# AlejandroSilvestri/os1

Measured on AMD Instinct MI355X. Metric: frames/sec extract+match, 1920x1080 @ 2000 ORB feats, higher is better.
Workload: dtype u8

## Files before the change

### os1_amd/csrc/orbfe_fast.hip

```cpp
#include <hip/hip_runtime.h>

#include <algorithm>
#include <cstdlib>
#include <type_traits>
#include <vector>

#include "orbfe_internal.h"

namespace orbfe {

namespace {
__device__ __forceinline__ int m24(int a, int b) { return __mul24(a, b); }
typedef unsigned short u16x2 __attribute__((ext_vector_type(2)));
__device__ __forceinline__ u16x2 as_u16x2(unsigned v) { return __builtin_bit_cast(u16x2, v); }
__device__ __forceinline__ unsigned as_u32(u16x2 v) { return __builtin_bit_cast(unsigned, v); }
}

__device__ __forceinline__ unsigned pk_min3_h(unsigned a, unsigned b, unsigned c) {
  unsigned r;
  asm("v_pk_minimum3_f16 %0, %1, %2, %3" : "=v"(r) : "v"(a), "v"(b), "v"(c));
  return r;
}
__device__ __forceinline__ unsigned pk_max3_h(unsigned a, unsigned b, unsigned c) {
  unsigned r;
  asm("v_pk_maximum3_f16 %0, %1, %2, %3" : "=v"(r) : "v"(a), "v"(b), "v"(c));
  return r;
}

__device__ __forceinline__ void wave_lds_fence() { asm volatile("s_waitcnt lgkmcnt(0)" ::: "memory"); }

struct FastArgs {
  const FastCell* cells;
  const uint8_t* const* frame0;
  const uint8_t* frameInline[2];
  long long stride0;
  uint8_t* slab;
  long long slabBytes;
  uint32_t* cellCount;
  uint32_t* slots;
  long long slotsPerFrame;
  const uint8_t* zeros;
  int ncells, pad, iniTh, minTh, frameBase;
};
static FastArgs fast_args(const PyramidParams& P) {
  FastArgs A{};
  A.cells = P.cells; A.frame0 = P.frame0; A.frameInline[0] = P.frameInline[0]; A.frameInline[1] = P.frameInline[1];
  A.stride0 = P.stride0; A.slab = P.slab; A.slabBytes = P.slabBytes; A.cellCount = P.cellCount; A.slots = P.slots;
  A.slotsPerFrame = P.slotsPerFrame; A.zeros = P.zeros; A.ncells = P.ncells; A.iniTh = P.iniTh; A.minTh = P.minTh;
  A.frameBase = P.frameBase;
  return A;
}

__device__ uint32_t* g_fastStampBuf;
template <int ABL = 0, bool LEAN = false>
__global__ __launch_bounds__(64) __attribute__((amdgpu_num_sgpr(96))) void k_fast_tasks(FastArgs P, int cb, int nc) {
  extern __shared__ __align__(16) uint8_t lds[];
  unsigned long long stamp[6] = {0, 0, 0, 0, 0, 0};
  if constexpr (ABL == 4) stamp[0] = __builtin_amdgcn_s_memtime();
  asm volatile("" ::"s"(P.cells), "s"(P.frame0), "s"(P.frameInline[0]), "s"(P.frameInline[1]), "s"(P.stride0), "s"(P.slab), "s"(P.slabBytes),
               "s"(P.cellCount), "s"(P.slots), "s"(P.slotsPerFrame), "s"(P.zeros), "s"(P.ncells), "s"(P.iniTh), "s"(P.minTh), "s"(P.frameBase),
               "s"(cb), "s"(nc));
  const int chunk = (nc + 7) >> 3;
  const int cloc = (blockIdx.x & 7) * chunk + (blockIdx.x >> 3);
  if (cloc >= nc) return;
  const int cix = cb + cloc;
  const int f = P.frameBase + blockIdx.y;
  const int lane = threadIdx.x;
  typedef uint32_t u32x8 __attribute__((ext_vector_type(8)));
  typedef uint32_t u32x2 __attribute__((ext_vector_type(2)));
  const u32x8 tw = *reinterpret_cast<const u32x8 __attribute__((address_space(4)))*>(reinterpret_cast<uintptr_t>(P.cells + cix));
  u32x2 fpw;
  if (P.frame0) {
    fpw = *reinterpret_cast<const u32x2 __attribute__((address_space(4)))*>(reinterpret_cast<uintptr_t>(P.frame0 + f));
  } else {
    const unsigned long long v = reinterpret_cast<unsigned long long>((f & 1) ? P.frameInline[1] : P.frameInline[0]);
    fpw.x = (uint32_t)v;
    fpw.y = (uint32_t)(v >> 32);
  }
  const int ex0 = (int)(tw[0] & 0xffffu), ey0 = (int)(tw[0] >> 16);
  const int ew = (int)(tw[1] & 0xffu), eh = (int)((tw[1] >> 16) & 0xffu), level = (int)(tw[1] >> 24);
  const uint32_t cell = tw[2], slotOff = tw[3], roiOff = tw[4], pitchL = tw[5];
  const int wCell = (int)(tw[6] & 0xffu), hCell = (int)((tw[6] >> 8) & 0xffu);
  uint32_t* cnt;
  if constexpr (LEAN) cnt = reinterpret_cast<uint32_t*>(reinterpret_cast<uint8_t*>(P.cellCount) + 4u * ((uint32_t)f * (uint32_t)P.ncells + cell));
  else cnt = P.cellCount + (long long)f * P.ncells + cell;
  if (ew == 0) {
    if (lane == 0) cnt[0] = 0;
    return;
  }
  long long stride;
  const uint8_t* roi;
  if constexpr (LEAN) {
    const bool l0 = level == 0;
    const uint32_t st32 = l0 ? (uint32_t)P.stride0 : pitchL;
    const uint32_t off = l0 ? (uint32_t)(ey0 - 3) * st32 + (uint32_t)(ex0 - 3) : (uint32_t)f * (uint32_t)P.slabBytes + roiOff;
    const uint8_t* base = l0 ? reinterpret_cast<const uint8_t*>(((unsigned long long)fpw.y << 32) | fpw.x) : P.slab;
    stride = (long long)st32;
    roi = base + off;
  } else if (level == 0) {
    stride = P.stride0;
    roi = reinterpret_cast<const uint8_t*>(((unsigned long long)fpw.y << 32) | fpw.x) + (long long)(ey0 - 3) * stride + (ex0 - 3);
  } else {
    stride = (long long)pitchL;
    roi = P.slab + (long long)f * P.slabBytes + roiOff;
  }
  const uint32_t geo = tw[7];
  const int TP = LEAN ? (int)(geo & 7u) << 4 : ((wCell + 6 + 3 + 15) & ~15);
  const int SP = wCell + 2;
  uint8_t* tile = lds;
  const int scOff = LEAN ? (int)((geo >> 8) & 0x3ffu) << 4 : (TP * (hCell + 6) + 15) & ~15;
  uint8_t* sc = tile + scOff;
  uint16_t* queue = reinterpret_cast<uint16_t*>(lds + (LEAN ? (int)((geo >> 18) & 0x7ffu) << 4 : ((scOff + SP * (hCell + 2) + 15) & ~15)));

  const int rw = ew + 6, rh = eh + 6;
  const int istr = (int)stride;
  const int a = (int)(reinterpret_cast<uintptr_t>(roi) & 3);
  if constexpr (ABL == 4) { asm volatile("" ::"s"(a), "s"(istr), "s"(TP) : "memory"); stamp[1] = __builtin_amdgcn_s_memtime(); }
  if constexpr (LEAN) {
    const int ppr = (int)(geo & 7u), rpi = (int)((geo >> 3) & 31u);
    const float rn = __builtin_amdgcn_rcpf((float)ppr);
    const int lrow = (int)(((float)lane + 0.5f) * rn), lcol = lane - m24(lrow, ppr);
    const bool on = lrow < rpi && 16 * lcol < a + rw;
    const unsigned voff = (unsigned)(m24(lrow, istr) + 16 * lcol);
    const uint8_t* gp = roi - a;
    const uint32_t gstep = (uint32_t)rpi * (uint32_t)istr;
    const int lstep = rpi * TP;
    uint8_t* lp = tile;
#pragma nounroll
    for (int left = rh; left > 0; left -= rpi, gp += gstep, lp += lstep) {
      unsigned vo = voff;
      asm volatile("" : "+s"(gp), "+v"(vo));
      if (on && lrow < left)
        __builtin_amdgcn_global_load_lds((const __attribute__((address_space(1))) void*)(gp + vo),
                                         (__attribute__((address_space(3))) void*)lp, 16, 0, 0);
    }
  } else if ((stride & 3) == 0) {
    const int ppr = TP >> 4;
    const float rn = __builtin_amdgcn_rcpf((float)ppr);
    const int rpi = 64 / ppr;
    const int lrow = (int)(((float)lane + 0.5f) * rn), lcol = lane - m24(lrow, ppr);
    const bool on = lrow < rpi && 16 * lcol < a + rw;
    const unsigned voff = (unsigned)(m24(lrow, istr) + 16 * lcol);
    const uint8_t* gp = roi - a;
    const long long gstep = (long long)rpi * stride;
    const int lstep = m24(rpi, TP);
    uint8_t* lp = tile;
    for (int left = rh; left > 0; left -= rpi, gp += gstep, lp += lstep) {
      unsigned vo = voff;
      asm volatile("" : "+s"(gp), "+v"(vo));
      if (on && lrow < left)
        __builtin_amdgcn_global_load_lds((const __attribute__((address_space(1))) void*)(gp + vo),
                                         (__attribute__((address_space(3))) void*)lp, 16, 0, 0);
    }
  } else {
    const float rcpRw = 1.0f / (float)rw;
    const int total = rw * rh;
    for (int i0 = lane; i0 < total; i0 += 64 * 8) {
      uint8_t v[8];
#pragma unroll
      for (int u = 0; u < 8; u++) {
        const int i = i0 + u * 64;
        v[u] = 0;
        if (i < total) {
          const int y = (int)(((float)i + 0.5f) * rcpRw), x = i - m24(y, rw);
          v[u] = roi[m24(y, istr) + x];
        }
      }
#pragma unroll
      for (int u = 0; u < 8; u++) {
        const int i = i0 + u * 64;
        if (i < total) {
          const int y = (int)(((float)i + 0.5f) * rcpRw), x = i - m24(y, rw);
          tile[m24(y, TP) + a + x] = v[u];
        }
      }
    }
  }
  tile += a;
  if constexpr (LEAN) {
    const int pieces = (SP * (eh + 2) + 15) >> 4;
#pragma nounroll
    for (int p0 = 0; p0 < pieces; p0 += 64)
      if (lane < pieces - p0)
        __builtin_amdgcn_global_load_lds((const __attribute__((address_space(1))) void*)P.zeros,
                                         (__attribute__((address_space(3))) void*)(sc + 16 * p0), 16, 0, 0);
  } else {
    const int pieces = (SP * (eh + 2) + 15) >> 4;
    for (int p0 = 0; p0 < pieces; p0 += 64)
      if (lane < pieces - p0)
        __builtin_amdgcn_global_load_lds((const __attribute__((address_space(1))) void*)P.zeros,
                                         (__attribute__((address_space(3))) void*)(sc + 16 * p0), 16, 0, 0);
  }
  asm volatile("s_waitcnt vmcnt(0)" ::: "memory");
  wave_lds_fence();
  if constexpr (ABL == 4) stamp[2] = __builtin_amdgcn_s_memtime();
  if constexpr (ABL == 1) {
    unsigned acc = 0;
    for (int i = lane; i < (TP * rh) >> 2; i += 64) acc ^= reinterpret_cast<const uint32_t*>(tile - a)[i];
    if (acc == 0x9e3779b9u && lane == 63) cnt[0] = 0;
    if (lane == 0) cnt[0] = 0;
    return;
  }

  const unsigned long long below = (1ull << lane) - 1ull;
  uint32_t* slot;
  if constexpr (LEAN) slot = reinterpret_cast<uint32_t*>(reinterpret_cast<uint8_t*>(P.slots) + 4u * ((uint32_t)f * (uint32_t)P.slotsPerFrame + slotOff));
  else slot = P.slots + (long long)f * P.slotsPerFrame + slotOff;
  int base = 0;
  for (int pass = 0; pass < 2; pass++) {
    const int tlo = pass ? P.minTh : P.iniTh;
    int nq = 0;
    constexpr int NPX = 16, GS = 4, NS = 4;
    const int G = (ew + NPX - 1) >> GS, nItems = G * eh;
    const int stepY = (int)((0x10152040u >> ((G - 1) << 3)) & 0xffu), stepG = 64 - stepY * G;
    auto stage1 = [&](auto aTag) {
      constexpr int A = decltype(aTag)::value;
      const u16x2 T2 = as_u16x2((unsigned)tlo * 0x01000100u);
      auto test4 = [&](uint32_t L4, uint32_t C4, uint32_t R4, uint32_t U4, uint32_t D4, unsigned& fe, unsigned& fo) {
        unsigned flag[2];
#pragma unroll
        for (int h = 0; h < 2; h++) {
          const u16x2 v2 = h ? as_u16x2(C4) << 8 : as_u16x2(C4);
          const u16x2 r0 = h ? as_u16x2(D4) << 8 : as_u16x2(D4), r4 = h ? as_u16x2(R4) << 8 : as_u16x2(R4);
          const u16x2 r8 = h ? as_u16x2(U4) << 8 : as_u16x2(U4), r12 = h ? as_u16x2(L4) << 8 : as_u16x2(L4);
          const u16x2 mx = __builtin_elementwise_min(__builtin_elementwise_max(r0, r8), __builtin_elementwise_max(r4, r12));
          const u16x2 mn = __builtin_elementwise_max(__builtin_elementwise_min(r0, r8), __builtin_elementwise_min(r4, r12));
          const u16x2 dd = __builtin_elementwise_max(__builtin_elementwise_sub_sat(mx, v2), __builtin_elementwise_sub_sat(v2, mn));
          const unsigned e = as_u32(__builtin_elementwise_sub_sat(dd, T2));
          asm("v_pk_min_u16 %0, %1, %2" : "=v"(flag[h]) : "v"(e), "v"(0x00010001u));
        }
        fo = flag[0];
        fe = flag[1];
      };
      int y = (int)(((float)lane + 0.5f) * __builtin_amdgcn_rcpf((float)G)), g = lane - m24(y, G);
      int ro = m24(y, TP) + (g << GS);
      const int roStep = m24(stepY, TP) + (stepG << GS), roCarry = TP - (G << GS);
      const uint8_t* tb = tile - a;
      for (int i0 = 0; i0 < nItems; i0 += 64) {
        unsigned m = 0;
        if (i0 + lane < nItems) {
          constexpr int c0 = (A + 3) >> 2, cs = (A + 3) & 3, q0 = (A + 6) >> 2, qs = (A + 6) & 3;
          const uint32_t* cw = reinterpret_cast<const uint32_t*>(tb + 3 * TP + ro);
          uint32_t w[NS + 3];
#pragma unroll
          for (int k = 0; k < NS + 3; k++) w[k] = cw[k];
          const uint32_t* uw = reinterpret_cast<const uint32_t*>(tb + ro) + c0;
          const uint32_t* dw = reinterpret_cast<const uint32_t*>(tb + 6 * TP + ro) + c0;
          uint32_t u[NS + 1], d[NS + 1];
#pragma unroll
          for (int k = 0; k < NS + 1; k++) { u[k] = uw[k]; d[k] = dw[k]; }
          unsigned E = 0, O = 0;
#pragma unroll
          for (int j = 0; j < NS; j++) {
            const uint32_t Lj = __builtin_amdgcn_alignbyte(w[j + 1], w[j], A);
            const uint32_t Cj = __builtin_amdgcn_alignbyte(w[c0 + j + 1], w[c0 + j], cs);
            const uint32_t Rj = __builtin_amdgcn_alignbyte(w[q0 + j + 1], w[q0 + j], qs);
            const uint32_t Uj = __builtin_amdgcn_alignbyte(u[j + 1], u[j], cs);
            const uint32_t Dj = __builtin_amdgcn_alignbyte(d[j + 1], d[j], cs);
            unsigned fe, fo;
            test4(Lj, Cj, Rj, Uj, Dj, fe, fo);
            E |= fe << (4 * j);
            O |= fo << (4 * j);
          }
          const unsigned T = E | (O << 1);
          const int rem = ew - (g << GS);
          m = (T | (T >> 14)) & ((1u << min(rem, NPX)) - 1u);
        }
        const int c = __popc(m);
        int incl = c;
        incl += __builtin_amdgcn_update_dpp(0, incl, 0x111, 0xf, 0xf, true);
        incl += __builtin_amdgcn_update_dpp(0, incl, 0x112, 0xf, 0xf, true);
        incl += __builtin_amdgcn_update_dpp(0, incl, 0x114, 0xf, 0xf, true);
        incl += __builtin_amdgcn_update_dpp(0, incl, 0x118, 0xf, 0xf, true);
        incl += __builtin_amdgcn_update_dpp(0, incl, 0x142, 0xa, 0xf, false);
        incl += __builtin_amdgcn_update_dpp(0, incl, 0x143, 0xc, 0xf, false);
        const int pos = nq + incl - c;
        const unsigned e = (unsigned)((y << 8) | (g << GS));
        {
          unsigned rev = __builtin_bitreverse32(m), ent = e;
          unsigned addr = (unsigned)(uintptr_t)(queue + pos);
          unsigned long long saved;
          asm volatile(
              "s_mov_b64 %3, exec\n\t"
              ".rept %4\n\t"
              "v_add_co_u32 %0, vcc, %0, %0\n\t"
              "s_and_b64 exec, %3, vcc\n\t"
              "ds_write_b16 %1, %2\n\t"
              "v_add_u32 %1, 2, %1\n\t"
              "s_mov_b64 exec, %3\n\t"
              "v_add_u32 %2, 1, %2\n\t"
              ".endr"
              : "+v"(rev), "+v"(addr), "+v"(ent), "=&s"(saved)
              : "n"(NPX)
              : "vcc", "scc", "memory");
        }
        nq += __builtin_amdgcn_readlane(incl, 63);
        if (i0 + 64 >= nItems) break;
        y += stepY;
        g += stepG;
        ro += roStep;
        if (g >= G) { g -= G; y++; ro += roCarry; }
      }
    };
    switch (a) {
      case 0: stage1(std::integral_constant<int, 0>{}); break;
      case 1: stage1(std::integral_constant<int, 1>{}); break;
      case 2: stage1(std::integral_constant<int, 2>{}); break;
      default: stage1(std::integral_constant<int, 3>{}); break;
    }
    wave_lds_fence();
    if constexpr (ABL == 4) { if (pass == 0) stamp[3] = __builtin_amdgcn_s_memtime(); }
    if constexpr (ABL == 2) {
      unsigned acc = 0;
      for (int i = lane; i < nq; i += 64) acc ^= queue[i];
      if (lane == 0) cnt[0] = (acc == 0xffffffffu) ? 1u : 0u;
      return;
    }
    int nq2 = 0;
    for (int i0 = 0; i0 < nq; i0 += 64) {
      const int i = i0 + lane;
      bool ok = false;
      unsigned e = 0;
      if (i < nq) {
        e = queue[i];
        const int y = e >> 8, x = e & 0xff;
        const uint8_t* c = tile + m24(y + 3, TP) + (x + 3);
        const unsigned vv = c[0];
        constexpr unsigned B = 2048u;
        unsigned xr[16];
        const unsigned VV = (B + vv) | ((B - vv) << 16);
#define RING(k, off) asm("v_pk_mad_i16 %0, %1, %2, %3 op_sel_hi:[0,1,1]" : "=v"(xr[k]) : "v"((unsigned)c[off]), "v"(0x0001ffffu), "v"(VV));
        RING(0, 3 * TP);       RING(1, 3 * TP + 1);   RING(2, 2 * TP + 2);    RING(3, TP + 3);
        RING(4, 3);            RING(5, -TP + 3);      RING(6, -2 * TP + 2);   RING(7, -3 * TP + 1);
        RING(8, -3 * TP);      RING(9, -3 * TP - 1);  RING(10, -2 * TP - 2);  RING(11, -TP - 3);
        RING(12, -3);          RING(13, TP - 3);      RING(14, 2 * TP - 2);   RING(15, 3 * TP - 1);
#undef RING
        unsigned t[16], arc[16];
#pragma unroll
        for (int k = 0; k < 16; k++) t[k] = pk_min3_h(xr[k], xr[(k + 1) & 15], xr[(k + 2) & 15]);
#pragma unroll
        for (int k = 0; k < 16; k++) arc[k] = pk_min3_h(t[k], t[(k + 3) & 15], t[(k + 6) & 15]);
        const unsigned m0 = pk_max3_h(arc[0], arc[1], arc[2]), m1 = pk_max3_h(arc[3], arc[4], arc[5]), m2 = pk_max3_h(arc[6], arc[7], arc[8]);
        const unsigned m3 = pk_max3_h(arc[9], arc[10], arc[11]), m4 = pk_max3_h(arc[12], arc[13], arc[14]);
        const unsigned best = pk_max3_h(pk_max3_h(m0, m1, m2), pk_max3_h(m3, m4, arc[15]), arc[15]);
        const int S = (int)max(best & 0xffffu, best >> 16) - (int)B;
        ok = S > tlo;
        if (ok) sc[m24(y + 1, SP) + (x + 1)] = (uint8_t)(S - 1);
      }
      const unsigned long long mk = __ballot(ok);
      if (ok) queue[nq2 + __popcll(mk & below)] = (uint16_t)e;
      nq2 += __popcll(mk);
    }
    wave_lds_fence();
    if constexpr (ABL == 4) { if (pass == 0) stamp[4] = __builtin_amdgcn_s_memtime(); }
    if constexpr (ABL == 3) {
      unsigned acc = 0;
      for (int i = lane; i < nq2; i += 64) acc ^= queue[i] ^ sc[i];
      if (lane == 0) cnt[0] = (acc == 0xffffffffu) ? 1u : 0u;
      return;
    }
    for (int i0 = 0; i0 < nq2; i0 += 64) {
      const int i = i0 + lane;
      int keep = 0, y = 0, x = 0;
      if (i < nq2) {
        const unsigned e = queue[i];
        y = e >> 8;
        x = e & 0xff;
        const uint8_t* q = sc + m24(y + 1, SP) + (x + 1);
        const int sv = q[0];
        const int nmax = max(max(max((int)q[-1], (int)q[-SP - 1]), (int)q[SP - 1]), max(max(max((int)q[1], (int)q[-SP + 1]), (int)q[SP + 1]), max((int)q[-SP], (int)q[SP])));
        if (sv > nmax) keep = sv;
      }
      const uint32_t rec = (uint32_t)(ex0 + x) | ((uint32_t)(ey0 + y) << 12) | ((uint32_t)keep << 24);
      const unsigned long long mk = __ballot(keep > 0);
      if (keep > 0) slot[base + __popcll(mk & below)] = rec;
      base += __popcll(mk);
    }
    if (pass == 1 || P.minTh == P.iniTh) break;
    if constexpr (ABL == 5) break;
    if (base != 0) break;
    wave_lds_fence();
  }
  if (lane == 0) cnt[0] = (uint32_t)base;
  if constexpr (ABL == 4) {
    stamp[5] = __builtin_amdgcn_s_memtime();
    if (lane == 0 && g_fastStampBuf) {
      uint32_t* rec = g_fastStampBuf + 8ull * ((unsigned long long)blockIdx.y * (P.ncells + 64) + cix);
      for (int k = 0; k < 5; k++) rec[k] = (uint32_t)(stamp[k + 1] - stamp[k]);
      rec[5] = 1u;
    }
  }
}

#ifdef ORBFE_EXPERIMENTS
static uint32_t* s_stampBuf = nullptr;
static size_t s_stampWaves = 0;
int fast_stamps(unsigned long long out[8], int reset) {
  for (int k = 0; k < 8; k++) out[k] = 0;
  if (!s_stampBuf || !s_stampWaves) return 0;
  std::vector<uint32_t> h(8 * s_stampWaves);
  if (hipMemcpy(h.data(), s_stampBuf, h.size() * 4, hipMemcpyDeviceToHost) != hipSuccess) return 1;
  for (size_t w = 0; w < s_stampWaves; w++)
    if (h[8 * w + 5]) {
      for (int k = 0; k < 5; k++) out[k] += h[8 * w + k];
      out[5]++;
    }
  if (reset && hipMemset(s_stampBuf, 0, h.size() * 4) != hipSuccess) return 1;
  return 0;
}
static void stamp_buffer_for(size_t waves) {
  if (waves > s_stampWaves) {
    if (s_stampBuf) (void)hipFree(s_stampBuf);
    s_stampBuf = nullptr;
    if (hipMalloc((void**)&s_stampBuf, waves * 32) != hipSuccess) { s_stampWaves = 0; return; }
    s_stampWaves = waves;
    (void)hipMemcpyToSymbol(HIP_SYMBOL(g_fastStampBuf), &s_stampBuf, sizeof s_stampBuf);
  }
  (void)hipMemset(s_stampBuf, 0, s_stampWaves * 32);
}
#else
int fast_stamps(unsigned long long out[8], int) {
  for (int k = 0; k < 8; k++) out[k] = 0;
  return 1;
}
#endif

static size_t fast_lds_bytes_level(const LevelGeom& L) {
  const size_t TP = (size_t)((L.wCell + 6 + 3 + 15) & ~15);
  const size_t scOff = (TP * (L.hCell + 6) + 15) & ~(size_t)15;
  const size_t b = ((scOff + (size_t)(L.wCell + 2) * (L.hCell + 2) + 15) & ~(size_t)15) +
                   2 * (size_t)L.wCell * L.hCell + 64;
  return (b + 15) & ~(size_t)15;
}
uint32_t fast_cell_geo(int wCell, int hCell) {
  const uint32_t TP = (uint32_t)((wCell + 6 + 3 + 15) & ~15), ppr = TP >> 4;
  if (ppr == 0 || ppr > 7) return 0u;
  const uint32_t rpi = 64u / ppr;
  const uint32_t scOff = (TP * (uint32_t)(hCell + 6) + 15u) & ~15u;
  const uint32_t qOff = (scOff + (uint32_t)(wCell + 2) * (uint32_t)(hCell + 2) + 15u) & ~15u;
  if (rpi > 31u || (scOff >> 4) > 0x3ffu || (qOff >> 4) > 0x7ffu) return 0u;
  return ppr | (rpi << 3) | ((scOff >> 4) << 8) | ((qOff >> 4) << 18);
}

void launch_fast(const PyramidParams& P, int nframes, hipStream_t st) {
  const FastArgs FA = fast_args(P);
  const int level0 = 0, level1 = P.nlevels;
  constexpr size_t kLdsFull = 5120;
  static const int leanEnv = [] { const char* e = getenv("ORBFE_FAST_LEAN"); return e ? atoi(e) : 1; }();
#ifdef ORBFE_EXPERIMENTS
  static const int ablate = [] { const char* e = ORBFE_EXP_ENV("ORBFE_FAST_ABLATE"); return e ? atoi(e) : 0; }();
#endif
  int l = level0;
  while (l < level1) {
    int e = l + 1;
    size_t need = fast_lds_bytes_level(P.lv[l]);
    if (nframes > 2) {
      const bool small = need <= kLdsFull;
      while (e < level1 && (fast_lds_bytes_level(P.lv[e]) <= kLdsFull) == small) { need = std::max(need, fast_lds_bytes_level(P.lv[e])); e++; }
    } else {
      while (e < level1) { need = std::max(need, fast_lds_bytes_level(P.lv[e])); e++; }
    }
    const int cb = P.lv[l].cellBase, nc = (e < P.nlevels ? P.lv[e].cellBase : P.ncells) - cb;
    l = e;
    if (nc <= 0) continue;
    const dim3 grid(8 * ((nc + 7) / 8), nframes);
    const unsigned long long frames = (unsigned long long)P.frameBase + (unsigned long long)nframes;
    const bool lean = leanEnv && P.fastLean && P.zeros && (P.stride0 & 3) == 0 && P.stride0 > 0 && P.stride0 < (1ll << 31) &&
                      frames * (unsigned long long)P.slabBytes < (1ull << 32) && frames * (unsigned long long)P.slotsPerFrame * 4ull < (1ull << 32) &&
                      frames * (unsigned long long)P.ncells * 4ull < (1ull << 32) &&
                      (unsigned long long)P.lv[0].h * (unsigned long long)P.stride0 < (1ull << 32);
#ifdef ORBFE_EXPERIMENTS
    if (ablate) {
      if (ablate == 4 && cb == 0) stamp_buffer_for((size_t)(P.ncells + 64) * nframes);
#define ORBFE_FAST_ABL(A)                                                                                              \
  do {                                                                                                                 \
    if (lean) hipLaunchKernelGGL((k_fast_tasks<A, true>), grid, dim3(64), need, st, FA, cb, nc);                       \
    else hipLaunchKernelGGL((k_fast_tasks<A, false>), grid, dim3(64), need, st, FA, cb, nc);                           \
  } while (0)
      switch (ablate) {
        case 1: ORBFE_FAST_ABL(1); break;
        case 2: ORBFE_FAST_ABL(2); break;
        case 3: ORBFE_FAST_ABL(3); break;
        case 4: ORBFE_FAST_ABL(4); break;
        default: ORBFE_FAST_ABL(5); break;
      }
#undef ORBFE_FAST_ABL
      continue;
    }
#endif
    if (lean) hipLaunchKernelGGL((k_fast_tasks<0, true>), grid, dim3(64), need, st, FA, cb, nc);
    else hipLaunchKernelGGL((k_fast_tasks<0, false>), grid, dim3(64), need, st, FA, cb, nc);
  }
}

}
```

Before: 89530.

## Pair FAST cells per two-wave block and pool tail scoring across waves

```diff
diff --git a/os1_amd/csrc/fast_pool_plan.h b/os1_amd/csrc/fast_pool_plan.h
--- /dev/null
+++ b/os1_amd/csrc/fast_pool_plan.h
@@ -0,0 +1,43 @@
+#pragma once
+
+#if defined(__HIPCC__) || defined(__CUDACC__)
+#define ORBFE_FAST_POOL_HD __host__ __device__
+#else
+#define ORBFE_FAST_POOL_HD
+#endif
+
+namespace orbfe {
+
+constexpr int kFastTrip = 64;
+enum FastPoolMode { kFastPoolNone = 0, kFastPoolPooled = 1, kFastPoolSeparate = 2 };
+
+struct FastPoolPlan {
+  int mode;
+  int la, lb;
+  int runner;
+  int sync;
+};
+
+ORBFE_FAST_POOL_HD inline FastPoolPlan fast_pool_plan(int nqA, int nqB) {
+  FastPoolPlan p;
+  p.la = nqA > kFastTrip ? nqA - kFastTrip : 0;
+  p.lb = nqB > kFastTrip ? nqB - kFastTrip : 0;
+  const int sum = p.la + p.lb;
+  p.mode = sum == 0 ? kFastPoolNone : sum <= kFastTrip ? kFastPoolPooled : kFastPoolSeparate;
+  p.sync = (p.mode == kFastPoolPooled && p.la > 0 && p.lb > 0) ? 1 : 0;
+  p.runner = (p.mode == kFastPoolPooled && p.la == 0) ? 1 : 0;
+  return p;
+}
+
+ORBFE_FAST_POOL_HD inline int fast_pool_own_end(const FastPoolPlan& p, int wave, int nq) {
+  if (p.mode == kFastPoolPooled && (p.sync || p.runner != wave)) return nq < kFastTrip ? nq : kFastTrip;
+  return nq;
+}
+
+ORBFE_FAST_POOL_HD inline bool fast_pool_lane(const FastPoolPlan& p, int lane, int& cell, int& entry) {
+  if (lane < p.la) { cell = 0; entry = kFastTrip + lane; return true; }
+  if (lane < p.la + p.lb) { cell = 1; entry = kFastTrip + lane - p.la; return true; }
+  return false;
+}
+
+}
diff --git a/os1_amd/csrc/orbfe_fast.hip b/os1_amd/csrc/orbfe_fast.hip
--- a/os1_amd/csrc/orbfe_fast.hip
+++ b/os1_amd/csrc/orbfe_fast.hip
@@ -5,6 +5,7 @@
 #include <type_traits>
 #include <vector>
 
+#include "fast_pool_plan.h"
 #include "orbfe_internal.h"
 
 namespace orbfe {
@@ -28,6 +29,7 @@
 }
 
 __device__ __forceinline__ void wave_lds_fence() { asm volatile("s_waitcnt lgkmcnt(0)" ::: "memory"); }
+__device__ __forceinline__ void block_sync() { asm volatile("s_waitcnt lgkmcnt(0)\n\ts_barrier" ::: "memory"); }
 
 struct FastArgs {
   const FastCell* cells;
@@ -53,19 +55,23 @@
 
 __device__ uint32_t* g_fastStampBuf;
 template <int ABL = 0, bool LEAN = false>
-__global__ __launch_bounds__(64) __attribute__((amdgpu_num_sgpr(96))) void k_fast_tasks(FastArgs P, int cb, int nc) {
+__global__ __launch_bounds__(128) __attribute__((amdgpu_num_sgpr(96))) void k_fast_tasks(FastArgs P, int cb, int nc, int need) {
   extern __shared__ __align__(16) uint8_t lds[];
   unsigned long long stamp[6] = {0, 0, 0, 0, 0, 0};
   if constexpr (ABL == 4) stamp[0] = __builtin_amdgcn_s_memtime();
   asm volatile("" ::"s"(P.cells), "s"(P.frame0), "s"(P.frameInline[0]), "s"(P.frameInline[1]), "s"(P.stride0), "s"(P.slab), "s"(P.slabBytes),
                "s"(P.cellCount), "s"(P.slots), "s"(P.slotsPerFrame), "s"(P.zeros), "s"(P.ncells), "s"(P.iniTh), "s"(P.minTh), "s"(P.frameBase),
-               "s"(cb), "s"(nc));
-  const int chunk = (nc + 7) >> 3;
-  const int cloc = (blockIdx.x & 7) * chunk + (blockIdx.x >> 3);
-  if (cloc >= nc) return;
-  const int cix = cb + cloc;
+               "s"(cb), "s"(nc), "s"(need));
+  const int np = (nc + 1) >> 1;
+  const int chunk = (np + 7) >> 3;
+  const int ploc = (blockIdx.x & 7) * chunk + (blockIdx.x >> 3);
+  if (ploc >= np) return;
+  const int wv = __builtin_amdgcn_readfirstlane((int)(threadIdx.x >> 6));
+  const int cloc = 2 * ploc + wv;
+  const bool have = cloc < nc;
+  const int cix = cb + (have ? cloc : nc - 1);
   const int f = P.frameBase + blockIdx.y;
-  const int lane = threadIdx.x;
+  const int lane = threadIdx.x & 63;
   typedef uint32_t u32x8 __attribute__((ext_vector_type(8)));
   typedef uint32_t u32x2 __attribute__((ext_vector_type(2)));
   const u32x8 tw = *reinterpret_cast<const u32x8 __attribute__((address_space(4)))*>(reinterpret_cast<uintptr_t>(P.cells + cix));
@@ -84,10 +90,7 @@
   uint32_t* cnt;
   if constexpr (LEAN) cnt = reinterpret_cast<uint32_t*>(reinterpret_cast<uint8_t*>(P.cellCount) + 4u * ((uint32_t)f * (uint32_t)P.ncells + cell));
   else cnt = P.cellCount + (long long)f * P.ncells + cell;
-  if (ew == 0) {
-    if (lane == 0) cnt[0] = 0;
-    return;
-  }
+  const bool active = have && ew != 0;
   long long stride;
   const uint8_t* roi;
   if constexpr (LEAN) {
@@ -107,16 +110,19 @@
   const uint32_t geo = tw[7];
   const int TP = LEAN ? (int)(geo & 7u) << 4 : ((wCell + 6 + 3 + 15) & ~15);
   const int SP = wCell + 2;
-  uint8_t* tile = lds;
+  uint8_t* const half = lds + wv * need;
+  uint32_t* const mbox = reinterpret_cast<uint32_t*>(lds + 2 * need);
+  uint8_t* tile = half;
   const int scOff = LEAN ? (int)((geo >> 8) & 0x3ffu) << 4 : (TP * (hCell + 6) + 15) & ~15;
   uint8_t* sc = tile + scOff;
-  uint16_t* queue = reinterpret_cast<uint16_t*>(lds + (LEAN ? (int)((geo >> 18) & 0x7ffu) << 4 : ((scOff + SP * (hCell + 2) + 15) & ~15)));
+  uint16_t* queue = reinterpret_cast<uint16_t*>(half + (LEAN ? (int)((geo >> 18) & 0x7ffu) << 4 : ((scOff + SP * (hCell + 2) + 15) & ~15)));
 
   const int rw = ew + 6, rh = eh + 6;
   const int istr = (int)stride;
   const int a = (int)(reinterpret_cast<uintptr_t>(roi) & 3);
   if constexpr (ABL == 4) { asm volatile("" ::"s"(a), "s"(istr), "s"(TP) : "memory"); stamp[1] = __builtin_amdgcn_s_memtime(); }
-  if constexpr (LEAN) {
+  if (!active) {
+  } else if constexpr (LEAN) {
     const int ppr = (int)(geo & 7u), rpi = (int)((geo >> 3) & 31u);
     const float rn = __builtin_amdgcn_rcpf((float)ppr);
     const int lrow = (int)(((float)lane + 0.5f) * rn), lcol = lane - m24(lrow, ppr);
@@ -177,7 +183,8 @@
     }
   }
   tile += a;
-  if constexpr (LEAN) {
+  if (!active) {
+  } else if constexpr (LEAN) {
     const int pieces = (SP * (eh + 2) + 15) >> 4;
 #pragma nounroll
     for (int p0 = 0; p0 < pieces; p0 += 64)
@@ -196,10 +203,18 @@
   if constexpr (ABL == 4) stamp[2] = __builtin_amdgcn_s_memtime();
   if constexpr (ABL == 1) {
     unsigned acc = 0;
-    for (int i = lane; i < (TP * rh) >> 2; i += 64) acc ^= reinterpret_cast<const uint32_t*>(tile - a)[i];
-    if (acc == 0x9e3779b9u && lane == 63) cnt[0] = 0;
-    if (lane == 0) cnt[0] = 0;
+    if (active)
+      for (int i = lane; i < (TP * rh) >> 2; i += 64) acc ^= reinterpret_cast<const uint32_t*>(tile - a)[i];
+    if (have && acc == 0x9e3779b9u && lane == 63) cnt[0] = 0;
+    if (have && lane == 0) cnt[0] = 0;
     return;
+  }
+  if (wv == 1 && lane == 0) {
+    mbox[8 + 3] = (uint32_t)(tile - lds);
+    mbox[8 + 4] = (uint32_t)TP;
+    mbox[8 + 5] = (uint32_t)(sc - lds);
+    mbox[8 + 6] = (uint32_t)SP;
+    mbox[8 + 7] = (uint32_t)(reinterpret_cast<uint8_t*>(queue) - lds);
   }
 
   const unsigned long long below = (1ull << lane) - 1ull;
@@ -207,12 +222,13 @@
   if constexpr (LEAN) slot = reinterpret_cast<uint32_t*>(reinterpret_cast<uint8_t*>(P.slots) + 4u * ((uint32_t)f * (uint32_t)P.slotsPerFrame + slotOff));
   else slot = P.slots + (long long)f * P.slotsPerFrame + slotOff;
   int base = 0;
+  bool mine = active;
   for (int pass = 0; pass < 2; pass++) {
     const int tlo = pass ? P.minTh : P.iniTh;
     int nq = 0;
     constexpr int NPX = 16, GS = 4, NS = 4;
     const int G = (ew + NPX - 1) >> GS, nItems = G * eh;
-    const int stepY = (int)((0x10152040u >> ((G - 1) << 3)) & 0xffu), stepG = 64 - stepY * G;
+    const int stepY = (int)((0x10152040u >> (((G - 1) & 3) << 3)) & 0xffu), stepG = 64 - stepY * G;
     auto stage1 = [&](auto aTag) {
       constexpr int A = decltype(aTag)::value;
       const u16x2 T2 = as_u16x2((unsigned)tlo * 0x01000100u);
@@ -302,7 +318,7 @@
         if (g >= G) { g -= G; y++; ro += roCarry; }
       }
     };
-    switch (a) {
+    if (mine) switch (a) {
       case 0: stage1(std::integral_constant<int, 0>{}); break;
       case 1: stage1(std::integral_constant<int, 1>{}); break;
       case 2: stage1(std::integral_constant<int, 2>{}); break;
@@ -313,50 +329,85 @@
     if constexpr (ABL == 2) {
       unsigned acc = 0;
       for (int i = lane; i < nq; i += 64) acc ^= queue[i];
-      if (lane == 0) cnt[0] = (acc == 0xffffffffu) ? 1u : 0u;
+      if (have && lane == 0) cnt[0] = (acc == 0xffffffffu) ? 1u : 0u;
       return;
     }
+    if (lane == 0) mbox[8 * wv] = (uint32_t)nq;
+    block_sync();
+    const int nqOther = __builtin_amdgcn_readfirstlane((int)mbox[8 * (wv ^ 1)]);
+    const FastPoolPlan plan = fast_pool_plan(wv ? nqOther : nq, wv ? nq : nqOther);
+    auto score = [&](unsigned e, const uint8_t* tl, int tp, uint8_t* scb, int sp) -> bool {
+      const int y = e >> 8, x = e & 0xff;
+      const uint8_t* c = tl + m24(y + 3, tp) + (x + 3);
+      const unsigned vv = c[0];
+      constexpr unsigned B = 2048u;
+      unsigned xr[16];
+      const unsigned VV = (B + vv) | ((B - vv) << 16);
+#define RING(k, off) asm("v_pk_mad_i16 %0, %1, %2, %3 op_sel_hi:[0,1,1]" : "=v"(xr[k]) : "v"((unsigned)c[off]), "v"(0x0001ffffu), "v"(VV));
+      RING(0, 3 * tp);       RING(1, 3 * tp + 1);   RING(2, 2 * tp + 2);    RING(3, tp + 3);
+      RING(4, 3);            RING(5, -tp + 3);      RING(6, -2 * tp + 2);   RING(7, -3 * tp + 1);
+      RING(8, -3 * tp);      RING(9, -3 * tp - 1);  RING(10, -2 * tp - 2);  RING(11, -tp - 3);
+      RING(12, -3);          RING(13, tp - 3);      RING(14, 2 * tp - 2);   RING(15, 3 * tp - 1);
+#undef RING
+      unsigned t[16], arc[16];
+#pragma unroll
+      for (int k = 0; k < 16; k++) t[k] = pk_min3_h(xr[k], xr[(k + 1) & 15], xr[(k + 2) & 15]);
+#pragma unroll
+      for (int k = 0; k < 16; k++) arc[k] = pk_min3_h(t[k], t[(k + 3) & 15], t[(k + 6) & 15]);
+      const unsigned m0 = pk_max3_h(arc[0], arc[1], arc[2]), m1 = pk_max3_h(arc[3], arc[4], arc[5]), m2 = pk_max3_h(arc[6], arc[7], arc[8]);
+      const unsigned m3 = pk_max3_h(arc[9], arc[10], arc[11]), m4 = pk_max3_h(arc[12], arc[13], arc[14]);
+      const unsigned best = pk_max3_h(pk_max3_h(m0, m1, m2), pk_max3_h(m3, m4, arc[15]), arc[15]);
+      const int S = (int)max(best & 0xffffu, best >> 16) - (int)B;
+      const bool ok = S > tlo;
+      if (ok) scb[m24(y + 1, sp) + (x + 1)] = (uint8_t)(S - 1);
+      return ok;
+    };
     int nq2 = 0;
-    for (int i0 = 0; i0 < nq; i0 += 64) {
+    const int ownEnd = fast_pool_own_end(plan, wv, nq);
+    for (int i0 = 0; i0 < ownEnd; i0 += 64) {
       const int i = i0 + lane;
       bool ok = false;
       unsigned e = 0;
-      if (i < nq) {
+      if (i < ownEnd) {
         e = queue[i];
-        const int y = e >> 8, x = e & 0xff;
-        const uint8_t* c = tile + m24(y + 3, TP) + (x + 3);
-        const unsigned vv = c[0];
-        constexpr unsigned B = 2048u;
-        unsigned xr[16];
-        const unsigned VV = (B + vv) | ((B - vv) << 16);
-#define RING(k, off) asm("v_pk_mad_i16 %0, %1, %2, %3 op_sel_hi:[0,1,1]" : "=v"(xr[k]) : "v"((unsigned)c[off]), "v"(0x0001ffffu), "v"(VV));
-        RING(0, 3 * TP);       RING(1, 3 * TP + 1);   RING(2, 2 * TP + 2);    RING(3, TP + 3);
-        RING(4, 3);            RING(5, -TP + 3);      RING(6, -2 * TP + 2);   RING(7, -3 * TP + 1);
-        RING(8, -3 * TP);      RING(9, -3 * TP - 1);  RING(10, -2 * TP - 2);  RING(11, -TP - 3);
-        RING(12, -3);          RING(13, TP - 3);      RING(14, 2 * TP - 2);   RING(15, 3 * TP - 1);
-#undef RING
-        unsigned t[16], arc[16];
-#pragma unroll
-        for (int k = 0; k < 16; k++) t[k] = pk_min3_h(xr[k], xr[(k + 1) & 15], xr[(k + 2) & 15]);
-#pragma unroll
-        for (int k = 0; k < 16; k++) arc[k] = pk_min3_h(t[k], t[(k + 3) & 15], t[(k + 6) & 15]);
-        const unsigned m0 = pk_max3_h(arc[0], arc[1], arc[2]), m1 = pk_max3_h(arc[3], arc[4], arc[5]), m2 = pk_max3_h(arc[6], arc[7], arc[8]);
-        const unsigned m3 = pk_max3_h(arc[9], arc[10], arc[11]), m4 = pk_max3_h(arc[12], arc[13], arc[14]);
-        const unsigned best = pk_max3_h(pk_max3_h(m0, m1, m2), pk_max3_h(m3, m4, arc[15]), arc[15]);
-        const int S = (int)max(best & 0xffffu, best >> 16) - (int)B;
-        ok = S > tlo;
-        if (ok) sc[m24(y + 1, SP) + (x + 1)] = (uint8_t)(S - 1);
+        ok = score(e, tile, TP, sc, SP);
       }
       const unsigned long long mk = __ballot(ok);
       if (ok) queue[nq2 + __popcll(mk & below)] = (uint16_t)e;
       nq2 += __popcll(mk);
+    }
+    if (plan.sync) {
+      if (lane == 0) mbox[8 * wv + 1] = (uint32_t)nq2;
+      block_sync();
+      if (wv == 0) {
+        const int tileB = __builtin_amdgcn_readfirstlane((int)mbox[8 + 3]), tpB = __builtin_amdgcn_readfirstlane((int)mbox[8 + 4]);
+        const int scB = __builtin_amdgcn_readfirstlane((int)mbox[8 + 5]), spB = __builtin_amdgcn_readfirstlane((int)mbox[8 + 6]);
+        const int quB = __builtin_amdgcn_readfirstlane((int)mbox[8 + 7]);
+        int nq2B = __builtin_amdgcn_readfirstlane((int)mbox[8 + 1]);
+        const bool isA = lane < plan.la, on = lane < plan.la + plan.lb;
+        uint16_t* const qu = reinterpret_cast<uint16_t*>(lds + (isA ? (int)(reinterpret_cast<uint8_t*>(queue) - lds) : quB));
+        bool ok = false;
+        unsigned e = 0;
+        if (on) {
+          e = qu[kFastTrip + lane - (isA ? 0 : plan.la)];
+          ok = score(e, lds + (isA ? (int)(tile - lds) : tileB), isA ? TP : tpB, lds + (isA ? (int)(sc - lds) : scB), isA ? SP : spB);
+        }
+        const unsigned long long mk = __ballot(ok), maskA = (1ull << plan.la) - 1ull;
+        const unsigned long long mkA = mk & maskA, mkB = mk & ~maskA;
+        if (ok) qu[(isA ? nq2 : nq2B) + __popcll((isA ? mkA : mkB) & below)] = (uint16_t)e;
+        nq2 += __popcll(mkA);
+        nq2B += __popcll(mkB);
+        if (lane == 0) mbox[8 + 1] = (uint32_t)nq2B;
+      }
+      block_sync();
+      if (wv == 1) nq2 = __builtin_amdgcn_readfirstlane((int)mbox[8 + 1]);
     }
     wave_lds_fence();
     if constexpr (ABL == 4) { if (pass == 0) stamp[4] = __builtin_amdgcn_s_memtime(); }
     if constexpr (ABL == 3) {
       unsigned acc = 0;
       for (int i = lane; i < nq2; i += 64) acc ^= queue[i] ^ sc[i];
-      if (lane == 0) cnt[0] = (acc == 0xffffffffu) ? 1u : 0u;
+      if (have && lane == 0) cnt[0] = (acc == 0xffffffffu) ? 1u : 0u;
       return;
     }
     for (int i0 = 0; i0 < nq2; i0 += 64) {
@@ -378,13 +429,16 @@
     }
     if (pass == 1 || P.minTh == P.iniTh) break;
     if constexpr (ABL == 5) break;
-    if (base != 0) break;
-    wave_lds_fence();
-  }
-  if (lane == 0) cnt[0] = (uint32_t)base;
+    const int want = (mine && base == 0) ? 1 : 0;
+    if (lane == 0) mbox[8 * wv + 2] = (uint32_t)want;
+    block_sync();
+    if (!(want | __builtin_amdgcn_readfirstlane((int)mbox[8 * (wv ^ 1) + 2]))) break;
+    mine = want != 0;
+  }
+  if (have && lane == 0) cnt[0] = (uint32_t)base;
   if constexpr (ABL == 4) {
     stamp[5] = __builtin_amdgcn_s_memtime();
-    if (lane == 0 && g_fastStampBuf) {
+    if (have && lane == 0 && g_fastStampBuf) {
       uint32_t* rec = g_fastStampBuf + 8ull * ((unsigned long long)blockIdx.y * (P.ncells + 64) + cix);
       for (int k = 0; k < 5; k++) rec[k] = (uint32_t)(stamp[k + 1] - stamp[k]);
       rec[5] = 1u;
@@ -463,7 +517,9 @@
     const int cb = P.lv[l].cellBase, nc = (e < P.nlevels ? P.lv[e].cellBase : P.ncells) - cb;
     l = e;
     if (nc <= 0) continue;
-    const dim3 grid(8 * ((nc + 7) / 8), nframes);
+    const int np = (nc + 1) / 2;
+    const dim3 grid(8 * ((np + 7) / 8), nframes);
+    const size_t ldsBytes = 2 * need + 64;
     const unsigned long long frames = (unsigned long long)P.frameBase + (unsigned long long)nframes;
     const bool lean = leanEnv && P.fastLean && P.zeros && (P.stride0 & 3) == 0 && P.stride0 > 0 && P.stride0 < (1ll << 31) &&
                       frames * (unsigned long long)P.slabBytes < (1ull << 32) && frames * (unsigned long long)P.slotsPerFrame * 4ull < (1ull << 32) &&
@@ -474,8 +530,8 @@
       if (ablate == 4 && cb == 0) stamp_buffer_for((size_t)(P.ncells + 64) * nframes);
 #define ORBFE_FAST_ABL(A)                                                                                              \
   do {                                                                                                                 \
-    if (lean) hipLaunchKernelGGL((k_fast_tasks<A, true>), grid, dim3(64), need, st, FA, cb, nc);                       \
-    else hipLaunchKernelGGL((k_fast_tasks<A, false>), grid, dim3(64), need, st, FA, cb, nc);                           \
+    if (lean) hipLaunchKernelGGL((k_fast_tasks<A, true>), grid, dim3(128), ldsBytes, st, FA, cb, nc, (int)need);       \
+    else hipLaunchKernelGGL((k_fast_tasks<A, false>), grid, dim3(128), ldsBytes, st, FA, cb, nc, (int)need);           \
   } while (0)
       switch (ablate) {
         case 1: ORBFE_FAST_ABL(1); break;
@@ -488,9 +544,9 @@
       continue;
     }
 #endif
-    if (lean) hipLaunchKernelGGL((k_fast_tasks<0, true>), grid, dim3(64), need, st, FA, cb, nc);
-    else hipLaunchKernelGGL((k_fast_tasks<0, false>), grid, dim3(64), need, st, FA, cb, nc);
-  }
-}
-
-}
+    if (lean) hipLaunchKernelGGL((k_fast_tasks<0, true>), grid, dim3(128), ldsBytes, st, FA, cb, nc, (int)need);
+    else hipLaunchKernelGGL((k_fast_tasks<0, false>), grid, dim3(128), ldsBytes, st, FA, cb, nc, (int)need);
+  }
+}
+
+}
```

Result: slower. 83970 (-6.2%).
